# mmottl/gpr

Hardware: AMD Instinct MI355X
Metric: FITC nLML+grad training-points/sec at n=1M m=2048 d=8 (higher is better)
Workload: dtype f64

## Files before the change

### gpr_amd/csrc/exp_fast.h

```cpp
#pragma once

namespace gprhip {

struct ExpK {
  double l2e, ln2hi, ln2lo, c[12];
};

#if defined(__HIP_DEVICE_COMPILE__)
#define GPRHIP_PIN_SGPR(v) asm volatile("" : "+s"(v))
#else
#define GPRHIP_PIN_SGPR(v) (void)0
#endif

__host__ __device__ __forceinline__ ExpK exp_consts() {
  ExpK k;
  k.l2e = 1.4426950408889634074;
  k.ln2hi = 6.93147180369123816490e-01;
  k.ln2lo = 1.90821492927058770002e-10;
  double f = 2.0;
  for (int i = 0; i < 12; ++i) {
    k.c[i] = 1.0 / f;
    f *= (double)(i + 3);
  }
  GPRHIP_PIN_SGPR(k.l2e);
  GPRHIP_PIN_SGPR(k.ln2hi);
  GPRHIP_PIN_SGPR(k.ln2lo);
#pragma unroll
  for (int i = 0; i < 12; ++i) GPRHIP_PIN_SGPR(k.c[i]);
  return k;
}

__host__ __device__ __forceinline__ double exp_fast(double x, const ExpK& k) {
  x = (x < -800.0) ? -800.0 : x;
  const double n = __builtin_rint(x * k.l2e);
  double r = __builtin_fma(-n, k.ln2hi, x);
  r = __builtin_fma(-n, k.ln2lo, r);
  double q = k.c[11];
#pragma unroll
  for (int i = 10; i >= 0; --i) q = __builtin_fma(q, r, k.c[i]);
  const double p = __builtin_fma(r * r, q, r);
  return __builtin_ldexp(1.0 + p, (int)n);
}

}
```

### gpr_amd/csrc/grad_mfma.hip

```cpp
#include "kernels.h"
#include "exp_fast.h"

namespace gprhip {

namespace {

typedef double gd4 __attribute__((ext_vector_type(4)));
__device__ __forceinline__ gd4 mfma4(double a, double b, gd4 c) {
  return __builtin_amdgcn_mfma_f64_16x16x4f64(a, b, c, 0, 0, 0);
}
__device__ __forceinline__ double wsum(double v) {
#pragma unroll
  for (int o = 32; o > 0; o >>= 1) v += __shfl_xor(v, o);
  return v;
}

constexpr int G_RC = 64;

template <int KS4, int DT, int BT, typename TS, bool KR = false>
__global__ __launch_bounds__(256, (DT + BT <= 4 && KS4 <= 8) ? 2 : 1) void grad_mfma_kernel(GradArgs<TS> a) {
  constexpr int DP = DT * 16, LDP = DP + 1;
  constexpr int BP = BT > 0 ? BT * 16 : 1, LDB = BP + 1;
  constexpr bool PF = (DT <= 2 && BT <= 2);
  constexpr int NBUF = PF ? 2 : 1;
  __shared__ double ps[KR ? 1 : NBUF * G_RC * LDP];
  __shared__ double bs[BT > 0 ? NBUF * G_RC * LDB : 1];
  __shared__ double pn[KR ? 1 : NBUF * G_RC];
  __shared__ double red[4][2];
  __shared__ double sh[DP];
  const int tid = threadIdx.x, lane = tid & 63, wv = tid >> 6;
  if (tid < DP) sh[tid] = (a.shift && tid < a.d) ? a.shift[tid] : 0.0;
  __syncthreads();
  const int l15 = lane & 15, lq = lane >> 4;
  const int cb = blockIdx.x * 128 + wv * 32;
  const ExpK ek = exp_consts();

  double zf[2][KS4], zn[2];
  bool live_c[2];
#pragma unroll
  for (int jt = 0; jt < 2; ++jt) {
    const int col = cb + jt * 16 + l15;
    live_c[jt] = col < a.m;
    double s2 = 0.0;
    if constexpr (!KR) {
#pragma unroll
      for (int s = 0; s < KS4; ++s) {
        const int k = 4 * s + lq;
        const double z = (live_c[jt] && k < a.d) ? a.Z[(int64_t)col * a.d + k] - sh[k] : 0.0;
        zf[jt][s] = z;
        s2 += z * z;
      }
      s2 += __shfl_xor(s2, 16);
      s2 += __shfl_xor(s2, 32);
    }
    zn[jt] = s2;
  }
  gd4 g[DT][2], gb[BT > 0 ? BT : 1][2];
#pragma unroll
  for (int t = 0; t < DT; ++t)
#pragma unroll
    for (int jt = 0; jt < 2; ++jt) g[t][jt] = (gd4){0, 0, 0, 0};
#pragma unroll
  for (int t = 0; t < (BT > 0 ? BT : 1); ++t)
#pragma unroll
    for (int jt = 0; jt < 2; ++jt) gb[t][jt] = (gd4){0, 0, 0, 0};
  double cs[2] = {0.0, 0.0}, sE = 0.0, sED = 0.0;

  const int r0 = blockIdx.y * a.slab;
  const int r1 = min(a.rows, r0 + a.slab);

  auto load_x = [&](int first, double (&xv)[2][4]) {
#pragma unroll
    for (int jt = 0; jt < 2; ++jt)
#pragma unroll
      for (int r = 0; r < 4; ++r) {
        const int row = first + lq + 4 * r;
        const int64_t off = (int64_t)row * a.mp + cb + jt * 16 + l15;
        if constexpr (KR) xv[jt][r] = (row < r1) ? (double)a.X[off] * (double)a.K[off] : 0.0;
        else xv[jt][r] = (row < r1) ? (double)a.X[off] : 0.0;
      }
  };
  auto tile = [&](const double* psb, const double* bsb, const double* pnb, int rb, int rt, const double (&xv)[2][4]) {
    double ev[2][4];
#pragma unroll
    for (int jt = 0; jt < 2; ++jt) {
      if constexpr (KR) {
#pragma unroll
        for (int r = 0; r < 4; ++r) {
          const double e = live_c[jt] ? xv[jt][r] : 0.0;
          ev[jt][r] = e;
          cs[jt] += e;
          sE += e;
        }
      } else {
        gd4 s4 = (gd4){0, 0, 0, 0};
#pragma unroll
        for (int s = 0; s < KS4; ++s) s4 = mfma4(psb[(rt * 16 + l15) * LDP + 4 * s + lq], zf[jt][s], s4);
#pragma unroll
        for (int r = 0; r < 4; ++r) {
          const int lr = rt * 16 + lq + 4 * r;
          const double dist = fmax(pnb[lr] + zn[jt] - 2.0 * s4[r], 0.0);
          const double kv = exp_fast(a.log_sf2 + a.inv_ell2_05 * dist, ek);
          const double e = (live_c[jt] && rb + lr < r1) ? xv[jt][r] * kv : 0.0;
          ev[jt][r] = e;
          cs[jt] += e;
          sE += e;
          sED += e * dist;
        }
      }
    }
#pragma unroll
    for (int r = 0; r < 4; ++r) {
      const int prow = (rt * 16 + 4 * r + lq);
      if (BT == 0) {
#pragma unroll
        for (int t = 0; t < DT; ++t) {
          const double ap = psb[prow * LDP + t * 16 + l15];
          g[t][0] = mfma4(ap, ev[0][r], g[t][0]);
          g[t][1] = mfma4(ap, ev[1][r], g[t][1]);
        }
      }
      if (BT > 0) {
#pragma unroll
        for (int t = 0; t < (BT > 0 ? BT : 1); ++t) {
          const double ab = bsb[prow * LDB + t * 16 + l15];
          gb[t][0] = mfma4(ab, ev[0][r], gb[t][0]);
          gb[t][1] = mfma4(ab, ev[1][r], gb[t][1]);
        }
      }
    }
  };

  if constexpr (PF) {
    constexpr int RPP = 256 / DP, NPV = G_RC / RPP;
    constexpr int RPB = 256 / BP, NBV = BT > 0 ? G_RC / RPB : 1;
    const int sr = tid / DP, sk = tid % DP;
    const int br_ = tid / BP, bk = tid % BP;
    double pv[NPV], bv[NBV];
    auto fetch_pts = [&](int rb) {
      if constexpr (!KR) {
#pragma unroll
        for (int j = 0; j < NPV; ++j) {
          const int row = rb + sr + RPP * j;
          pv[j] = (sk < a.d && row < r1) ? a.pts[(int64_t)row * a.d + sk] - sh[sk] : 0.0;
        }
      }
      if constexpr (BT > 0) {
#pragma unroll
        for (int j = 0; j < NBV; ++j) {
          const int row = rb + br_ + RPB * j;
          bv[j] = (bk < a.D && row < r1) ? a.big[(int64_t)row * a.D + bk] : 0.0;
        }
      }
    };
    auto store_pts = [&](int buf) {
      if constexpr (!KR) {
#pragma unroll
        for (int j = 0; j < NPV; ++j) {
          const int r = sr + RPP * j;
          ps[buf * G_RC * LDP + r * LDP + sk] = pv[j];
          double s2 = pv[j] * pv[j];
          s2 += __shfl_xor(s2, 1);
          s2 += __shfl_xor(s2, 2);
          s2 += __shfl_xor(s2, 4);
          s2 += __shfl_xor(s2, 8);
          if constexpr (DP == 32) s2 += __shfl_xor(s2, 16);
          if (sk == 0) pn[buf * G_RC + r] = s2;
        }
      }
      if constexpr (BT > 0) {
#pragma unroll
        for (int j = 0; j < NBV; ++j) bs[buf * G_RC * LDB + (br_ + RPB * j) * LDB + bk] = bv[j];
      }
    };
    double xv[2][4], xn[2][4];
    fetch_pts(r0);
    load_x(r0, xv);
    store_pts(0);
    __syncthreads();
    int buf = 0;
    for (int rb = r0; rb < r1; rb += G_RC, buf ^= 1) {
      const bool more = rb + G_RC < r1;
      if (more) fetch_pts(rb + G_RC);
#pragma unroll 1
      for (int rt = 0; rt < G_RC / 16; ++rt) {
        if (rb + rt * 16 >= r1) break;
        load_x(rb + rt * 16 + 16, xn);
        tile(ps + buf * G_RC * LDP, bs + (BT > 0 ? buf * G_RC * LDB : 0), pn + buf * G_RC, rb, rt, xv);
#pragma unroll
        for (int jt = 0; jt < 2; ++jt)
#pragma unroll
          for (int r = 0; r < 4; ++r) xv[jt][r] = xn[jt][r];
      }
      if (more) store_pts(buf ^ 1);
      __syncthreads();
    }
  } else {
    for (int rb = r0; rb < r1; rb += G_RC) {
      __syncthreads();
      if constexpr (!KR) {
        for (int idx = tid; idx < G_RC * DP; idx += 256) {
          const int r = idx / DP, k = idx % DP;
          ps[r * LDP + k] = (k < a.d && rb + r < r1) ? a.pts[(int64_t)(rb + r) * a.d + k] - sh[k] : 0.0;
        }
      }
      if (BT > 0) {
        for (int idx = tid; idx < G_RC * BP; idx += 256) {
          const int r = idx / BP, k = idx % BP;
          bs[r * LDB + k] = (k < a.D && rb + r < r1) ? a.big[(int64_t)(rb + r) * a.D + k] : 0.0;
        }
      }
      __syncthreads();
      if constexpr (!KR) {
        if (tid < G_RC) {
          double s2 = 0.0;
          for (int k = 0; k < DP; ++k) s2 += ps[tid * LDP + k] * ps[tid * LDP + k];
          pn[tid] = s2;
        }
        __syncthreads();
      }
#pragma unroll 1
      for (int rt = 0; rt < G_RC / 16; ++rt) {
        if (rb + rt * 16 >= r1) break;
        double xv[2][4];
        load_x(rb + rt * 16, xv);
        tile(ps, bs, pn, rb, rt, xv);
      }
    }
  }

  double* cp = a.colpart + (int64_t)blockIdx.y * a.col_rows * a.mp;
#pragma unroll
  for (int jt = 0; jt < 2; ++jt) {
    const int col = cb + jt * 16 + l15;
    double c = cs[jt];
    c += __shfl_xor(c, 16);
    c += __shfl_xor(c, 32);
    if (lq == 0) cp[col] = c;
#pragma unroll
    for (int t = 0; t < DT; ++t)
#pragma unroll
      for (int r = 0; r < 4; ++r) {
        const int dim = t * 16 + lq + 4 * r;
        if (dim < a.d) cp[(int64_t)(1 + dim) * a.mp + col] = (BT == 0) ? g[t][jt][r] + sh[dim] * c : 0.0;
      }
    if (BT > 0) {
#pragma unroll
      for (int t = 0; t < (BT > 0 ? BT : 1); ++t)
#pragma unroll
        for (int r = 0; r < 4; ++r) {
          const int dim = t * 16 + lq + 4 * r;
          if (dim < a.D) cp[(int64_t)(a.d + 1 + dim) * a.mp + col] = gb[t][jt][r];
        }
    }
  }
  sE = wsum(sE);
  sED = wsum(sED);
  if (lane == 0) {
    red[wv][0] = sE;
    red[wv][1] = sED;
  }
  __syncthreads();
  if (tid < 2)
    a.scalpart[((int64_t)blockIdx.y * gridDim.x + blockIdx.x) * 2 + tid] =
        (red[0][tid] + red[1][tid]) + (red[2][tid] + red[3][tid]);
}

template <int KS4, int DT, typename TS>
void dispatch_big(const GradArgs<TS>& a, dim3 grid, hipStream_t s) {
  if (a.K && a.big) {
    if (a.D <= 16) hipLaunchKernelGGL((grad_mfma_kernel<KS4, DT, 1, TS, true>), grid, dim3(256), 0, s, a);
    else if (a.D <= 32) hipLaunchKernelGGL((grad_mfma_kernel<KS4, DT, 2, TS, true>), grid, dim3(256), 0, s, a);
    else hipLaunchKernelGGL((grad_mfma_kernel<KS4, DT, 4, TS, true>), grid, dim3(256), 0, s, a);
    return;
  }
  if (!a.big) hipLaunchKernelGGL((grad_mfma_kernel<KS4, DT, 0, TS>), grid, dim3(256), 0, s, a);
  else if (a.D <= 16) hipLaunchKernelGGL((grad_mfma_kernel<KS4, DT, 1, TS>), grid, dim3(256), 0, s, a);
  else if (a.D <= 32) hipLaunchKernelGGL((grad_mfma_kernel<KS4, DT, 2, TS>), grid, dim3(256), 0, s, a);
  else hipLaunchKernelGGL((grad_mfma_kernel<KS4, DT, 4, TS>), grid, dim3(256), 0, s, a);
}

}

template <typename TS>
int grad_mfma_col_blocks(const GradArgs<TS>& a) {
  if (a.ms || a.d > 64 || a.D > 64 || (a.mp % 128) != 0) return 0;
  return a.mp / 128;
}

template <typename TS>
void launch_grad_mfma(const GradArgs<TS>& a, hipStream_t s) {
  dim3 grid(a.mp / 128, (a.rows + a.slab - 1) / a.slab);
  if (a.d <= 4) dispatch_big<1, 1, TS>(a, grid, s);
  else if (a.d <= 8) dispatch_big<2, 1, TS>(a, grid, s);
  else if (a.d <= 16) dispatch_big<4, 1, TS>(a, grid, s);
  else if (a.d <= 32) dispatch_big<8, 2, TS>(a, grid, s);
  else dispatch_big<16, 4, TS>(a, grid, s);
  GPR_HIP(hipGetLastError());
}

__global__ __launch_bounds__(256) void proj_inducing_grad_kernel(double* __restrict__ acc, int mp, int d, int D,
                                                                 const double* __restrict__ tproj) {
  const int c = blockIdx.x * 256 + threadIdx.x, k = blockIdx.y;
  if (c >= mp) return;
  double s = 0.0;
  for (int b = 0; b < D; ++b) s += tproj[(int64_t)k * D + b] * acc[(int64_t)(d + 1 + b) * mp + c];
  acc[(int64_t)(1 + k) * mp + c] += s;
}
void launch_proj_inducing_grad(double* acc, int mp, int d, int D, const double* tproj, hipStream_t s) {
  hipLaunchKernelGGL(proj_inducing_grad_kernel, dim3((mp + 255) / 256, d), dim3(256), 0, s, acc, mp, d, D, tproj);
  GPR_HIP(hipGetLastError());
}

template int grad_mfma_col_blocks<double>(const GradArgs<double>&);
template int grad_mfma_col_blocks<float>(const GradArgs<float>&);
template void launch_grad_mfma<double>(const GradArgs<double>&, hipStream_t);
template void launch_grad_mfma<float>(const GradArgs<float>&, hipStream_t);

}
```

Measured before the change: 2.790 million.

## Interleave exp evaluations, unroll row tiles by two, and clamp loads branch-free

Adds a batched exp_fast_n that evaluates four exponentials in lockstep so their FMA chains overlap, and issues both column-tile MFMA distance products before the exp work when IL holds. The inner row-tile loop is unrolled by two with ping-pong x buffers, which removes the register copy and lets the next loads overlap the current tile. Global loads now clamp indices instead of predicating them, with masking moved to the shared-memory store. The cost is higher register pressure, which could lower occupancy, plus some redundant loads at slab edges.

```diff
diff --git a/gpr_amd/csrc/exp_fast.h b/gpr_amd/csrc/exp_fast.h
--- a/gpr_amd/csrc/exp_fast.h
+++ b/gpr_amd/csrc/exp_fast.h
@@ -42,4 +42,25 @@
   return __builtin_ldexp(1.0 + p, (int)n);
 }
 
+template <int N>
+__host__ __device__ __forceinline__ void exp_fast_n(double (&x)[N], const ExpK& k) {
+  double n[N], r[N], q[N];
+#pragma unroll
+  for (int j = 0; j < N; ++j) x[j] = (x[j] < -800.0) ? -800.0 : x[j];
+#pragma unroll
+  for (int j = 0; j < N; ++j) n[j] = __builtin_rint(x[j] * k.l2e);
+#pragma unroll
+  for (int j = 0; j < N; ++j) r[j] = __builtin_fma(-n[j], k.ln2hi, x[j]);
+#pragma unroll
+  for (int j = 0; j < N; ++j) r[j] = __builtin_fma(-n[j], k.ln2lo, r[j]);
+#pragma unroll
+  for (int j = 0; j < N; ++j) q[j] = k.c[11];
+#pragma unroll
+  for (int i = 10; i >= 0; --i)
+#pragma unroll
+    for (int j = 0; j < N; ++j) q[j] = __builtin_fma(q[j], r[j], k.c[i]);
+#pragma unroll
+  for (int j = 0; j < N; ++j) x[j] = __builtin_ldexp(1.0 + __builtin_fma(r[j] * r[j], q[j], r[j]), (int)n[j]);
 }
+
+}
diff --git a/gpr_amd/csrc/grad_mfma.hip b/gpr_amd/csrc/grad_mfma.hip
--- a/gpr_amd/csrc/grad_mfma.hip
+++ b/gpr_amd/csrc/grad_mfma.hip
@@ -23,6 +23,7 @@
   constexpr int BP = BT > 0 ? BT * 16 : 1, LDB = BP + 1;
   constexpr bool PF = (DT <= 2 && BT <= 2);
   constexpr int NBUF = PF ? 2 : 1;
+  constexpr bool IL = PF && (KS4 <= 2 || BT == 0);
   __shared__ double ps[KR ? 1 : NBUF * G_RC * LDP];
   __shared__ double bs[BT > 0 ? NBUF * G_RC * LDB : 1];
   __shared__ double pn[KR ? 1 : NBUF * G_RC];
@@ -75,16 +76,26 @@
 #pragma unroll
       for (int r = 0; r < 4; ++r) {
         const int row = first + lq + 4 * r;
-        const int64_t off = (int64_t)row * a.mp + cb + jt * 16 + l15;
-        if constexpr (KR) xv[jt][r] = (row < r1) ? (double)a.X[off] * (double)a.K[off] : 0.0;
-        else xv[jt][r] = (row < r1) ? (double)a.X[off] : 0.0;
+        if constexpr (!PF) {
+          const int64_t o = (int64_t)row * a.mp + cb + jt * 16 + l15;
+          if constexpr (KR) xv[jt][r] = (row < r1) ? (double)a.X[o] * (double)a.K[o] : 0.0;
+          else xv[jt][r] = (row < r1) ? (double)a.X[o] : 0.0;
+          continue;
+        }
+        const int64_t off = (int64_t)min(row, r1 - 1) * a.mp + cb + jt * 16 + l15;
+        if constexpr (KR) {
+          const double e = (double)a.X[off] * (double)a.K[off];
+          xv[jt][r] = (row < r1) ? e : 0.0;
+        } else {
+          xv[jt][r] = (double)a.X[off];
+        }
       }
   };
   auto tile = [&](const double* psb, const double* bsb, const double* pnb, int rb, int rt, const double (&xv)[2][4]) {
     double ev[2][4];
-#pragma unroll
-    for (int jt = 0; jt < 2; ++jt) {
-      if constexpr (KR) {
+    if constexpr (KR) {
+#pragma unroll
+      for (int jt = 0; jt < 2; ++jt)
 #pragma unroll
         for (int r = 0; r < 4; ++r) {
           const double e = live_c[jt] ? xv[jt][r] : 0.0;
@@ -92,20 +103,39 @@
           cs[jt] += e;
           sE += e;
         }
-      } else {
-        gd4 s4 = (gd4){0, 0, 0, 0};
-#pragma unroll
-        for (int s = 0; s < KS4; ++s) s4 = mfma4(psb[(rt * 16 + l15) * LDP + 4 * s + lq], zf[jt][s], s4);
+    } else {
+      gd4 s4[2];
+      if constexpr (IL) {
+#pragma unroll
+        for (int jt = 0; jt < 2; ++jt) {
+          s4[jt] = (gd4){0, 0, 0, 0};
+#pragma unroll
+          for (int s = 0; s < KS4; ++s) s4[jt] = mfma4(psb[(rt * 16 + l15) * LDP + 4 * s + lq], zf[jt][s], s4[jt]);
+        }
+      }
+#pragma unroll
+      for (int jt = 0; jt < 2; ++jt) {
+        if constexpr (!IL) {
+          s4[jt] = (gd4){0, 0, 0, 0};
+#pragma unroll
+          for (int s = 0; s < KS4; ++s) s4[jt] = mfma4(psb[(rt * 16 + l15) * LDP + 4 * s + lq], zf[jt][s], s4[jt]);
+        }
+        double dist[4], kv[4];
+#pragma unroll
+        for (int r = 0; r < 4; ++r) {
+          dist[r] = fmax(pnb[rt * 16 + lq + 4 * r] + zn[jt] - 2.0 * s4[jt][r], 0.0);
+          kv[r] = a.log_sf2 + a.inv_ell2_05 * dist[r];
+          if constexpr (!IL) kv[r] = exp_fast(kv[r], ek);
+        }
+        if constexpr (IL) exp_fast_n<4>(kv, ek);
 #pragma unroll
         for (int r = 0; r < 4; ++r) {
           const int lr = rt * 16 + lq + 4 * r;
-          const double dist = fmax(pnb[lr] + zn[jt] - 2.0 * s4[r], 0.0);
-          const double kv = exp_fast(a.log_sf2 + a.inv_ell2_05 * dist, ek);
-          const double e = (live_c[jt] && rb + lr < r1) ? xv[jt][r] * kv : 0.0;
+          const double e = (live_c[jt] && rb + lr < r1) ? xv[jt][r] * kv[r] : 0.0;
           ev[jt][r] = e;
           cs[jt] += e;
           sE += e;
-          sED += e * dist;
+          sED += e * dist[r];
         }
       }
     }
@@ -140,26 +170,23 @@
     auto fetch_pts = [&](int rb) {
       if constexpr (!KR) {
 #pragma unroll
-        for (int j = 0; j < NPV; ++j) {
-          const int row = rb + sr + RPP * j;
-          pv[j] = (sk < a.d && row < r1) ? a.pts[(int64_t)row * a.d + sk] - sh[sk] : 0.0;
-        }
+        for (int j = 0; j < NPV; ++j)
+          pv[j] = a.pts[(int64_t)min(rb + sr + RPP * j, r1 - 1) * a.d + min(sk, a.d - 1)];
       }
       if constexpr (BT > 0) {
 #pragma unroll
-        for (int j = 0; j < NBV; ++j) {
-          const int row = rb + br_ + RPB * j;
-          bv[j] = (bk < a.D && row < r1) ? a.big[(int64_t)row * a.D + bk] : 0.0;
-        }
+        for (int j = 0; j < NBV; ++j)
+          bv[j] = a.big[(int64_t)min(rb + br_ + RPB * j, r1 - 1) * a.D + min(bk, a.D - 1)];
       }
     };
-    auto store_pts = [&](int buf) {
+    auto store_pts = [&](int rb, int buf) {
       if constexpr (!KR) {
 #pragma unroll
         for (int j = 0; j < NPV; ++j) {
           const int r = sr + RPP * j;
-          ps[buf * G_RC * LDP + r * LDP + sk] = pv[j];
-          double s2 = pv[j] * pv[j];
+          const double pj = (sk < a.d && rb + r < r1) ? pv[j] - sh[sk] : 0.0;
+          ps[buf * G_RC * LDP + r * LDP + sk] = pj;
+          double s2 = pj * pj;
           s2 += __shfl_xor(s2, 1);
           s2 += __shfl_xor(s2, 2);
           s2 += __shfl_xor(s2, 4);
@@ -170,29 +197,33 @@
       }
       if constexpr (BT > 0) {
 #pragma unroll
-        for (int j = 0; j < NBV; ++j) bs[buf * G_RC * LDB + (br_ + RPB * j) * LDB + bk] = bv[j];
+        for (int j = 0; j < NBV; ++j) {
+          const int r = br_ + RPB * j;
+          bs[buf * G_RC * LDB + r * LDB + bk] = (bk < a.D && rb + r < r1) ? bv[j] : 0.0;
+        }
       }
     };
-    double xv[2][4], xn[2][4];
+    double xa[2][4], xb[2][4];
     fetch_pts(r0);
-    load_x(r0, xv);
-    store_pts(0);
+    load_x(r0, xa);
+    store_pts(r0, 0);
     __syncthreads();
     int buf = 0;
     for (int rb = r0; rb < r1; rb += G_RC, buf ^= 1) {
       const bool more = rb + G_RC < r1;
       if (more) fetch_pts(rb + G_RC);
+      const double* psb = ps + buf * G_RC * LDP;
+      const double* bsb = bs + (BT > 0 ? buf * G_RC * LDB : 0);
+      const double* pnb = pn + buf * G_RC;
 #pragma unroll 1
-      for (int rt = 0; rt < G_RC / 16; ++rt) {
+      for (int rt = 0; rt < G_RC / 16; rt += 2) {
         if (rb + rt * 16 >= r1) break;
-        load_x(rb + rt * 16 + 16, xn);
-        tile(ps + buf * G_RC * LDP, bs + (BT > 0 ? buf * G_RC * LDB : 0), pn + buf * G_RC, rb, rt, xv);
-#pragma unroll
-        for (int jt = 0; jt < 2; ++jt)
-#pragma unroll
-          for (int r = 0; r < 4; ++r) xv[jt][r] = xn[jt][r];
-      }
-      if (more) store_pts(buf ^ 1);
+        load_x(rb + rt * 16 + 16, xb);
+        tile(psb, bsb, pnb, rb, rt, xa);
+        load_x(rb + rt * 16 + 32, xa);
+        if (rb + rt * 16 + 16 < r1) tile(psb, bsb, pnb, rb, rt + 1, xb);
+      }
+      if (more) store_pts(rb + G_RC, buf ^ 1);
       __syncthreads();
     }
   } else {
```

New measurement: 2.795 million (median of 6 runs). Within noise of the previous version (+0.2%).
